# mohakbhardwaj/mjmpc

Hardware: AMD Instinct MI355X
Metric: particle-steps/sec (reacher_7dof-v0 MPPI 4096p x H32 per GPU, control loop incl. noise, rollout, update, shift) (higher is better)
Workload: dtype f64

## Files before the change

include/mjmpc_amd.h:

```cpp
#ifndef MJMPC_AMD_H
#define MJMPC_AMD_H

#include <stdint.h>

#ifdef __cplusplus
extern "C" {
#endif

#define MJMPC_ABI_VERSION 4

#define MJMPC_F32 0
#define MJMPC_F64 1

#define MJMPC_E_BADARG (-1)
#define MJMPC_E_BADMODEL (-2)
#define MJMPC_E_NOGPU (-3)

#define MJMPC_ARM_BLOB_LEN 255
#define MJMPC_ARM_STATE_LEN 19

typedef struct mjmpc_arm_s* mjmpc_arm_t;

int mjmpc_abi_version(void);
const char* mjmpc_last_error(void);
int mjmpc_device_count(void);
int mjmpc_graph_kernel_nodes(void* hip_graph, int64_t* n_out);
int mjmpc_graph_signature(void* hip_graph, uint64_t* n_out);

int mjmpc_arm_create(const double* model_blob, int n_blob, int device, mjmpc_arm_t* out);
int mjmpc_arm_destroy(mjmpc_arm_t h);
int mjmpc_arm_dims(mjmpc_arm_t h, int* nv, int* nu, int* d_obs);

int mjmpc_arm_set_shard_models(mjmpc_arm_t h, const double* model_blobs, int n_shards);

int mjmpc_arm_set_state(mjmpc_arm_t h, const double* qpos, const double* qvel, const double* target_pos,
                        void* stream);
int mjmpc_arm_set_shard_states(mjmpc_arm_t h, const double* states, int n_shards, void* stream);
double* mjmpc_arm_state_ptr(mjmpc_arm_t h);

int mjmpc_arm_rollout(mjmpc_arm_t h, int dtype, int64_t P, int H, const double* d_mean, const void* d_noise,
                      void* d_costs, void* d_actions, void* d_obs, void* d_next_obs, void* stream);

int mjmpc_arm_rollout_cl(mjmpc_arm_t h, int dtype, int64_t P, int H, const double* d_weights, const void* d_noise,
                         void* d_costs, void* d_actions, void* d_obs, void* d_next_obs, void* stream);

int mjmpc_arm_rollout_fused(mjmpc_arm_t h, int dtype, int64_t P, int H, const double* d_mean, const void* d_noise,
                            const double* d_filter_coeffs, const double* d_gseq, void* d_costs, void* d_actions,
                            double* d_q0, void* stream);

int mjmpc_arm_mppi_step(mjmpc_arm_t h, int dtype, int64_t P, int H, const double* d_mean, double* d_mean_out,
                        const double* d_gseq, const double* d_filter_coeffs, const double* d_chol, uint64_t seed,
                        uint64_t offset, int64_t particle_offset, int64_t* d_step_counter, double lam, double step_size,
                        int shift_mode, double* d_action_out, double* h_action_slots, double* d_record, int env_step,
                        void* d_step_cost, void* d_step_next_obs, void* d_costs, void* d_actions, double* d_q0, void* stream);

int mjmpc_arm_rollout_sampled(mjmpc_arm_t h, int dtype, int64_t P, int H, const double* d_mean, const double* d_gseq,
                              const double* d_filter_coeffs, const double* d_chol, int chol_full, uint64_t seed, uint64_t offset,
                              int64_t particle_offset, const int64_t* d_step_counter, void* d_costs, void* d_actions,
                              double* d_q0, void* stream);

int mjmpc_arm_mppi_combine(mjmpc_arm_t h, int dtype, const double* d_records, int n_records, int H, const double* d_mean,
                           double* d_mean_out, int64_t* d_step_counter, double step_size, int shift_mode,
                           double* d_action_out, double* h_action_slots, int env_step, void* d_step_cost,
                           void* d_step_next_obs, void* stream);

int mjmpc_arm_step_state(mjmpc_arm_t h, int dtype, const double* d_action, void* d_cost, void* d_next_obs,
                         void* stream);
int mjmpc_arm_get_state(mjmpc_arm_t h, double* qpos, double* qvel, void* stream);
int mjmpc_arm_rollout_fused_batch(mjmpc_arm_t h, int dtype, int64_t P_total, int H, const double* d_means, const void* d_noise,
                                  const double* d_filter_coeffs, const double* d_gseq, void* d_costs, void* d_actions,
                                  double* d_q0, void* stream);
int mjmpc_arm_rollout_fused_batch_obs(mjmpc_arm_t h, int dtype, int64_t P_total, int H, const double* d_means,
                                      const void* d_noise, const double* d_filter_coeffs, const double* d_gseq, void* d_costs,
                                      void* d_actions, double* d_q0, void* d_next_obs, void* stream);
int mjmpc_arm_step_shard_states(mjmpc_arm_t h, int dtype, const double* d_actions, void* d_costs, void* d_next_obs, void* stream);
int mjmpc_arm_get_shard_states(mjmpc_arm_t h, double* qpos, double* qvel, void* stream);

// ... 266 lines not shown
```

mjmpc_amd/_lib.py:

```python
import ctypes
import os
import threading

_HERE = os.path.dirname(os.path.abspath(__file__))
LIB_PATH = os.environ.get("MJMPC_AMD_LIB", os.path.join(_HERE, "libmjmpc_amd.so"))

F32, F64 = 0, 1
ABI_VERSION = 4

_vp = ctypes.c_void_p
_i64 = ctypes.c_int64
_int = ctypes.c_int
_dbl = ctypes.c_double
_dp = ctypes.POINTER(ctypes.c_double)

SIGNATURES = {
    "mjmpc_abi_version": (_int, []),
    "mjmpc_last_error": (ctypes.c_char_p, []),
    "mjmpc_device_count": (_int, []),
    "mjmpc_arm_create": (_int, [_dp, _int, _int, ctypes.POINTER(_vp)]),
    "mjmpc_arm_set_shard_models": (_int, [_vp, _dp, _int]),
    "mjmpc_arm_set_shard_states": (_int, [_vp, _dp, _int, _vp]),
    "mjmpc_arm_destroy": (_int, [_vp]),
    "mjmpc_arm_dims": (_int, [_vp, ctypes.POINTER(_int), ctypes.POINTER(_int), ctypes.POINTER(_int)]),
    "mjmpc_arm_set_state": (_int, [_vp, _dp, _dp, _dp, _vp]),
    "mjmpc_arm_state_ptr": (_vp, [_vp]),
    "mjmpc_arm_rollout": (_int, [_vp, _int, _i64, _int, _vp, _vp, _vp, _vp, _vp, _vp, _vp]),
    "mjmpc_arm_rollout_cl": (_int, [_vp, _int, _i64, _int, _vp, _vp, _vp, _vp, _vp, _vp, _vp]),
    "mjmpc_arm_rollout_fused": (_int, [_vp, _int, _i64, _int, _vp, _vp, _vp, _vp, _vp, _vp, _vp, _vp]),
    "mjmpc_tree_rollout_fused": (_int, [_vp, _int, _i64, _int, _vp, _vp, _vp, _vp, _vp, _vp, _vp, _vp]),
    "mjmpc_arm_step_state": (_int, [_vp, _int, _vp, _vp, _vp, _vp]),
    "mjmpc_arm_get_state": (_int, [_vp, _dp, _dp, _vp]),
    "mjmpc_arm_rollout_fused_batch": (_int, [_vp, _int, _i64, _int, _vp, _vp, _vp, _vp, _vp, _vp, _vp, _vp]),
    "mjmpc_arm_rollout_fused_batch_obs": (_int, [_vp, _int, _i64, _int, _vp, _vp, _vp, _vp, _vp, _vp, _vp, _vp, _vp]),
    "mjmpc_arm_step_shard_states": (_int, [_vp, _int, _vp, _vp, _vp, _vp]),
    "mjmpc_arm_get_shard_states": (_int, [_vp, _dp, _dp, _vp]),
    "mjmpc_arm_mppi_combine": (_int, [_vp, _int, _vp, _int, _int, _vp, _vp, _vp, ctypes.c_double, _int, _vp, _vp, _int, _vp, _vp, _vp]),
    "mjmpc_arm_rollout_sampled": (_int, [_vp, _int, _i64, _int, _vp, _vp, _vp, _vp, _int, ctypes.c_uint64, ctypes.c_uint64, _i64, _vp,
                                         _vp, _vp, _vp, _vp]),
    "mjmpc_arm_mppi_step": (_int, [_vp, _int, _i64, _int, _vp, _vp, _vp, _vp, _vp, ctypes.c_uint64, ctypes.c_uint64, _i64, _vp,
                                   _dbl, _dbl, _int, _vp, _vp, _vp, _int, _vp, _vp, _vp, _vp, _vp, _vp]),
    "mjmpc_tree_create": (_int, [_dp, _int, _int, ctypes.POINTER(_vp)]),
    "mjmpc_tree_create_ex": (_int, [_dp, _int, _int, _int, ctypes.POINTER(_vp)]),
    "mjmpc_tree_destroy": (_int, [_vp]),
    "mjmpc_tree_dims": (_int, [_vp, ctypes.POINTER(_int), ctypes.POINTER(_int), ctypes.POINTER(_int)]),
    "mjmpc_tree_nq": (_int, [_vp]),
    "mjmpc_tree_set_shard_models": (_int, [_vp, _dp, _int]),
    "mjmpc_tree_set_state": (_int, [_vp, _dp, _dp, _dp, _vp]),
    "mjmpc_tree_set_shard_states": (_int, [_vp, _dp, _int, _vp]),
    "mjmpc_tree_rollout": (_int, [_vp, _int, _i64, _int, _vp, _vp, _vp, _vp, _vp, _vp, _vp]),
    "mjmpc_tree_rollout_cl": (_int, [_vp, _int, _i64, _int, _vp, _vp, _vp, _vp, _vp, _vp, _vp]),
    "mjmpc_tree_step_state": (_int, [_vp, _int, _vp, _vp, _vp, _vp]),
    "mjmpc_tree_get_state": (_int, [_vp, _dp, _dp, _vp]),
    "mjmpc_tree_rollout_fused_batch": (_int, [_vp, _int, _i64, _int, _vp, _vp, _vp, _vp, _vp, _vp, _vp, _vp]),
    "mjmpc_tree_rollout_fused_batch_obs": (_int, [_vp, _int, _i64, _int, _vp, _vp, _vp, _vp, _vp, _vp, _vp, _vp, _vp]),
    "mjmpc_tree_step_shard_states": (_int, [_vp, _int, _vp, _vp, _vp, _vp]),
    "mjmpc_tree_get_shard_states": (_int, [_vp, _dp, _dp, _vp]),
    "mjmpc_tree_set_batch_models": (_int, [_vp, _dp, _int, _int]),
    "mjmpc_tree_set_env_model": (_int, [_vp, _dp]),
    "mjmpc_tree_solver_failures": (_int, [_vp, ctypes.POINTER(ctypes.c_uint32)]),
    "mjmpc_tree_diverged": (_int, [_vp, ctypes.POINTER(ctypes.c_uint32)]),
    "mjmpc_analytic_rollout": (_int, [_int, _vp, _int, _int, _vp, _int, _i64, _int, _vp, _vp, _vp, _vp, _vp, _vp, _int,
                                      _vp]),
    "mjmpc_arm_solver_failures": (_int, [_vp, ctypes.POINTER(ctypes.c_uint32)]),
# ... 181 lines not shown
```

mjmpc_amd/control/controller.py:

```python
import copy
import ctypes
import gc
import inspect
from abc import ABC, abstractmethod

import numpy as np

from .. import _lib
from ._device import DeviceUpdater
from .sharding import local_block
from .control_utils import generate_noise


def _seed_value(seed):
    if seed is None:
        seed = int(np.random.SeedSequence().generate_state(1)[0])
    if not isinstance(seed, (int, np.integer)) or seed < 0:
        raise ValueError("Seed must be a non-negative integer or omitted, not {}".format(seed))
    return int(seed)


class Controller(ABC):
    def __init__(self, d_state, d_obs, d_action, action_lows, action_highs, horizon, gamma, n_iters,
                 set_sim_state_fn=None, rollout_fn=None, sample_mode='mean', batch_size=1, seed=0,
# ... 314 lines not shown
        if self.noise_mode == 'device_mt19937':
            return self.dev.sample_noise_mt19937(n_loc, self._cov_host, self.filter_coeffs, self.seed_val, steps_ahead,
                                                 dtype=self.noise_dtype, d_step=self._step_dev, filtered=False,
                                                 particle_offset=self.dev.comm.rank * n_loc)
        return self.dev.sample_noise(n_loc, self._noise_cov(), self.filter_coeffs, self.seed_val, steps_ahead,
                                     dtype=self.noise_dtype, d_step=self._step_dev, filtered=False,
                                     particle_offset=self.dev.comm.rank * n_loc,
                                     device_cov_diagonal=self.cov_type == 'diagonal')

    def _noise_cov(self):
        return self._cov_host if self._static_cov() else None

    def _bind_mono(self, env_step, direct=False):
        n_loc = self.local_particles
        chol, coeffs, _ = self.dev.prepare_noise(self._cov_host, self.filter_coeffs)
        fc = np.asarray(self.filter_coeffs, np.float64)
        coeffs = None if (fc[0] == 1.0 and fc[1] == 0.0 and fc[2] == 0.0) else coeffs
        eng = getattr(self._rollout_fn, "engine", None)
        post = self._graph_post
        own_step = post is not None and getattr(post, "__self__", None) is eng and getattr(post, "__name__", "") == "step_state"
        sharded = self.dev.comm.world_size > 1
        self._mono_rec = self.dev.record("fused_rec", 2 + self.horizon * self.d_action) if sharded else None
        self._mono_steps_env = bool(env_step and own_step)
        self._mono_launch, self._mono_combine = {}, {}
        recs = self.dev.comm.all_gather(self._mono_rec) if sharded else None
        self._mono_gather = None
        if sharded:
            mk = getattr(self.dev.comm, "all_gather_launcher", None)
            self._mono_gather = mk(self._mono_rec) if (mk and direct) else (lambda: self.dev.comm.all_gather(self._mono_rec))
        for src, dst in ((self.dev.mean, self.dev.mean_alt), (self.dev.mean_alt, self.dev.mean)):
            self._mono_launch[id(src)], _ = self._rollout_fn.mono_launcher(
                n_loc, self.horizon, src, dst, self.dev.gseq, coeffs, chol, self.seed_val, 0, self.dev.comm.rank * n_loc,
                self._step_dev, self.lam, self.step_size, _SHIFT_MODES[self.base_action], action_out=self._action_dev,
                action_slots=None if sharded else self._action_pin, record=self._mono_rec,
                env_step=self._mono_steps_env and not sharded,
                bind_stream=direct or not sharded)
            if sharded:
                self._mono_combine[id(src)] = self._rollout_fn.combine_launcher(
                    recs, recs.shape[0], self.horizon, src, dst, self._step_dev, self.step_size,
                    _SHIFT_MODES[self.base_action], self._action_dev, self._action_pin, self._mono_steps_env)

    def _noise_ahead(self):
        return ((not self._mono) and self._graph_on and self.noise_mode == 'device'
                and (self._fused_capable() or (self._cem_fused() and not self._cem_in_kernel())))

    def _cem_in_kernel(self):
        eng = getattr(self._rollout_fn, "engine", None)
        return (self._cem_fused() and getattr(self, "_want_cem_in_kernel", True) and hasattr(self._rollout_fn, "sampled")
                and hasattr(eng, "mppi_step_supported") and eng.mppi_step_supported(self.local_particles, self.horizon)
                and getattr(eng, "num_shards", 1) == 1 and not getattr(eng, "_per_shard_states", False)
                and not hasattr(eng, "shard_blobs") and getattr(eng, "dtype", self.noise_dtype) == self.noise_dtype)

    def _cem_fused(self):
        return False

    def _mono_capable(self):
        if not (getattr(self, "_want_mono", True) and self._graph_on and self.noise_mode == 'device' and self.n_iters == 1
                and self._fused_capable() and self._static_cov() and hasattr(self._rollout_fn, "mono")):
            return False
# ... 107 lines not shown
            self._step_host = self.num_steps
            self._action_dev = torch.zeros(self.d_action, dtype=torch.float64, device=self.dev.device)
            self._action_pin = torch.zeros(2 * (self.d_action + 1), dtype=torch.float64).pin_memory()
            self._action_np = self._action_pin.numpy()
            if self._mono and (self.dev.comm.world_size == 1 or getattr(self.dev.comm, "lib_collectives", False)):
                self._bind_mono(env_step=True, direct=True)
                self._graph = "direct"
                self.launch_mode = "launched directly"
            else:
                self._capture_iteration()
        if self._graph is None:
            return self._optimize_eager_after_fallback(state)
        if self._step_host != self.num_steps:
            if self._ahead:
                raise RuntimeError("num_steps was changed while an iteration enqueued ahead was in flight")
            self._step_dev.fill_(self.num_steps)
            self._noise_valid = False
        if not self._noise_valid:
            if self._noise_ahead():
                self._draw_raw(self.local_particles, 0)
            elif self._cem_in_kernel():
                self.dev.factor_cov(self.filter_coeffs)
            self._noise_valid = True
        replay = self._device_iteration if self._graph == "direct" else self._graph.replay
        if self._ahead == 0:
            self._action_np[self._slot(self.num_steps) + self.d_action] = -1.0
            replay()
            self._ahead = 1
        if self._lookahead and self._mono and self.dev.comm.world_size == 1:
            self._action_np[self._slot(self.num_steps + 1) + self.d_action] = -1.0
            replay()
            self._ahead += 1
        action = self._wait_action()
        self._ahead -= 1
        self.num_steps += 1
        self._step_host = self.num_steps
        self._mean_stale = True
        if not self._static_cov():
            self._cov_stale = True
        return action, 0.0

    def _capture_iteration(self):
        torch = self.dev.torch
        sharded_mono = self._mono and self.dev.comm.world_size > 1
        if self._mono:
            self._bind_mono(env_step=False)
# ... 39 lines not shown
                    self._device_iteration()
                self._graph = self._tape_or_graph(g, tape, cap_stream)
            else:
                g = torch.cuda.CUDAGraph()
                with torch.cuda.graph(g):
                    self._device_iteration()
                self._graph = g
        except Exception as e:
            err = e
        finally:
            if gc_was_on:
                gc.enable()
        if not self.dev.comm.all_agree(err is None, self.dev.device):
            import warnings
            warnings.warn("hipGraph capture of the control iteration failed (%s); running eagerly"
                          % (err if err is not None else "on another rank",))
            torch.cuda.synchronize(self.dev.device)
            self.dev.mean.copy_(keep[0])
            self.dev.cov.copy_(keep[2])
            self._graph_on = False
            self._graph = None
            self.graph_fallback = True
            self._mono = False
            self._mono_launch, self._mono_combine = {}, {}

    def _tape_or_graph(self, g, tape, cap_stream):
        torch = self.dev.torch
        self.launch_mode = "hipGraph replay"
        try:
            t = _LaunchTape(tape, cap_stream, self.dev)
            g2 = torch.cuda.CUDAGraph(keep_graph=True)
            with torch.cuda.graph(g2):
                t.replay()
            n1, n2 = (ctypes.c_int64 * 2)(), (ctypes.c_int64 * 2)()
            _lib.check(self.dev.lib.mjmpc_graph_kernel_nodes(ctypes.c_void_p(int(g.raw_cuda_graph())), n1))
            _lib.check(self.dev.lib.mjmpc_graph_kernel_nodes(ctypes.c_void_p(int(g2.raw_cuda_graph())), n2))
            s1, s2 = (ctypes.c_uint64 * 2)(), (ctypes.c_uint64 * 2)()
            _lib.check(self.dev.lib.mjmpc_graph_signature(ctypes.c_void_p(int(g.raw_cuda_graph())), s1))
            _lib.check(self.dev.lib.mjmpc_graph_signature(ctypes.c_void_p(int(g2.raw_cuda_graph())), s2))
            del g2
            if n1[0] > 0 and n1[0] == n2[0] and n1[1] == n2[1] and s1[0] == s2[0] and s1[1] == s2[1]:
                self.launch_mode = "launch tape (%d calls, %d kernels)" % (len(t.calls), n1[0])
                return t
        except Exception as e:
            import warnings
            warnings.warn("launch tape not available (%s); replaying the hipGraph" % (e,))
        g.instantiate()
# ... 57 lines not shown
```

mjmpc_amd/csrc/arm_rollout.hip:

```cpp
#include <hip/hip_runtime.h>

#include <cstdlib>
#include <type_traits>

#include "arm_model.h"
#include "arm_rollout.h"
#include "lanegroup.h"
#include "noise_device.h"

namespace mjmpc {
namespace {

template <typename T>
constexpr int newton_maxit() { return sizeof(T) == 4 ? 32 : 12; }

#define PHASE() asm volatile("" ::: "memory")
#define LDS_WAVE_SYNC()                                        \
    do {                                                       \
        __builtin_amdgcn_fence(__ATOMIC_ACQ_REL, "wavefront"); \
        asm volatile("" ::: "memory");                         \
        __builtin_amdgcn_sched_barrier(0);                     \
    } while (0)

constexpr int N_LINK_FIELDS = O_NV / LANES;
// ... 1331 lines not shown
            const unsigned long long mine = particle_lanes(lane);
            const double* rst = record();
            if (rst == nullptr) {
            } else if (__ballot(mj_is_bad(x)) & mine) {
                q = (T)rst[l8];
                v = (T)rst[LANES + l8];
                sq = (T)rst[2 * LANES + 3 + l8];
                cq = (T)rst[3 * LANES + 3 + l8];
                aw = T(0);
                const int f0 = rflags<ROLE>(ldsM);
                rflags_set<ROLE>(ldsM, f0 | 1 | 4 | RST_EVER);
                if (role_counts<ROLE>() && diag && l8 == 0 && rc->count) { atomicAdd(diag + 1, 1u); if (f0 & RST_REAL) atomicAdd(diag + 2, 1u); }
            } else if (bal & mine) {
                rflags_set<ROLE>(ldsM, rflags<ROLE>(ldsM) | 2);
            }
        }
    }
    LDS_WAVE_SYNC();
    ST.mark(13);
}

constexpr int MONO_RED = 32;

template <typename T, bool DUO, typename MT>
__device__ __forceinline__ void real_env_step(const MT& M, const ArmInts& I, const MonoStep& mo, double* st, T q, T v,
                                              const T* tgt, const double* action, int A, T* lds, int lane, int wave, int l8,
                                              int g, unsigned* diag) {
    const int nv = I.nv;
    T* ldsM = lds + g * PSTRIDE;
    T aw = T(0);
    if (l8 >= nv) { q = T(0); v = T(0); }
    T sinq, cosq;
    sincos_(q, sinq, cosq);
    if constexpr (XJ) { if (M.xj_slide()) { sinq = T(0); cosq = T(1); } }
    int rows = 0;
    Stamps ST;
    ST.begin();
    bool fs = false;
    ResetCtl rc;
    rc.count = g == 0;
    if (DUO && wave == 1) rflags_set<SOLVE>(ldsM, RST_REAL);
    else rflags_set<SOLO>(ldsM, RST_REAL);
    auto record = [&mo]() -> const double* { return mo.reset_rec; };
    if (mo.reset_rec) {
        if (DUO && wave == 1) reset_check_start<SOLVE>(rc, q, v, lane, ldsM);
        else reset_check_start<SOLO>(rc, q, v, lane, ldsM);
    }
    if (DUO && wave == 1) {
        if constexpr (DUO) {
            T nosite[3];
            for (int sub = 0; sub < I.frame_skip; ++sub) {
                arm_front<SOLVE>(M, I, q, v, aw, sinq, cosq, rows, T(0), ldsM, lane, l8, nosite, diag, fs, ST, &rc);
                arm_back<SOLVE>(M, q, v, aw, sinq, cosq, ldsM, l8, fs, ST, lane, &rc, nullptr, record);
            }
        }
        return;
    }
    constexpr int R = DUO ? DYN : SOLO;
    const T u = l8 < A ? (T)action[l8] : T(0);
    const T tau_act = M.link(O_GEAR) * fmin(fmax(u, M.link(O_CTRL_LO)), M.link(O_CTRL_HI));
    T site[3];
    unsigned* dcount = diag;
    for (int sub = 0; sub < I.frame_skip; ++sub) {
        if (R == DYN && sub > 0) arm_back<R>(M, q, v, aw, sinq, cosq, ldsM, l8, fs, ST, lane, &rc, dcount, record);
        arm_front<R>(M, I, q, v, aw, sinq, cosq, rows, tau_act, ldsM, lane, l8, site, dcount, fs, ST, &rc);
        if constexpr (R == SOLO) arm_back<R>(M, q, v, aw, sinq, cosq, ldsM, l8, fs, ST, lane, &rc, dcount, record);
    }
    const int site_lane = lane_of_link(lane, I.site_link);
    for (int k = 0; k < 3; ++k) site[k] = __shfl(site[k], site_lane);
    if constexpr (R == DYN) arm_back<R>(M, q, v, aw, sinq, cosq, ldsM, l8, fs, ST, lane, &rc, dcount, record);
    if (rc.any && (rflags<R>(ldsM) & 4))
        for (int k = 0; k < 3; ++k) site[k] = (T)mo.reset_rec[2 * LANES + k];
    if (g == 0) {
        const T dx = site[0] - tgt[0], dy = site[1] - tgt[1], dz = site[2] - tgt[2];
        if (mo.step_cost && l8 == 0)
            ((T*)mo.step_cost)[0] = fabs(dx) + fabs(dy) + fabs(dz) + T(5) * sqrt_(dx * dx + dy * dy + dz * dz);
        if (mo.step_nobs) {
            T* o = (T*)mo.step_nobs;
            if (l8 < nv) { o[l8] = q; o[nv + l8] = v; }
            if (l8 < 3) {
                const T hh = l8 == 0 ? site[0] : (l8 == 1 ? site[1] : site[2]);
                const T gg = l8 == 0 ? tgt[0] : (l8 == 1 ? tgt[1] : tgt[2]);
// ... 16 lines not shown
        const double q = red[tid], x = q == INFINITY ? -INFINITY : (-1.0 / lam) * q;
        double m = x;
        for (int o = 1; o < LANES; o <<= 1) m = fmax(m, __shfl_xor(m, o));
        const double e = x == -INFINITY ? 0.0 : exp(x - m);
        double S = e;
        for (int o = 1; o < LANES; o <<= 1) S += __shfl_xor(S, o);
        red[LANES + tid] = e;
        if (tid == 0) { rec_out[0] = m; rec_out[1] = S; }
    }
    __syncthreads();
    double e[LANES];
#pragma unroll
    for (int k = 0; k < LANES; ++k) e[k] = red[LANES + k];
    for (int j = tid; j < HA; j += NT) {
        double acc = 0.0;
#pragma unroll
        for (int k = 0; k < LANES; ++k) acc += e[k] * (double)actT[k * HA + j];
        rec_out[2 + j] = acc;
    }
}

constexpr int MAX_A = 8;
constexpr int FIN_CHUNK = 4;
#ifdef MJMPC_ARM_XJ
#define MJMPC_FINISH_WAVES __attribute__((amdgpu_waves_per_eu(1, 1)))
#else
#define MJMPC_FINISH_WAVES
#endif
template <typename T>
__global__ __launch_bounds__(128) MJMPC_FINISH_WAVES void arm_mppi_finish_kernel(const T* __restrict__ model, const double* __restrict__ recs, long n_rec,
                                                              int H, int A, const double* __restrict__ mean_in,
                                                              double* __restrict__ mean_out, const MonoStep mo,
                                                              int env_step, unsigned* diag) {
    __shared__ __attribute__((aligned(16))) T lds[LANES * PSTRIDE + ARM_BLOB_LEN + 3];
    __shared__ double sh[2 * (2 + MAX_A)];
    const int tid = threadIdx.x, t = blockIdx.x, HA = H * A, rec = 2 + HA;
    const int lane = tid & 63, wave = __builtin_amdgcn_readfirstlane(tid >> 6);
    const bool stepper = t == 0 && env_step && mo.state_io && !mo.record;
    double rm[FIN_CHUNK], rs[FIN_CHUNK], rw[FIN_CHUNK][MAX_A];
    auto fetch = [&](long base) {
#pragma unroll
        for (int k = 0; k < FIN_CHUNK; ++k) {
            const long b = base + tid + 128L * k;
            const double* r = recs + (b < n_rec ? b : 0) * rec;
            rm[k] = b < n_rec ? r[0] : -INFINITY;
            rs[k] = r[1];
#pragma unroll
            for (int a = 0; a < MAX_A; ++a) rw[k][a] = a < A ? r[2 + t * A + a] : 0.0;
        }
    };
    fetch(0);
    const double mean_old = (tid < A && !mo.record) ? mean_in[t * A + tid] : 0.0;
    const long long count = (t == 0 && mo.step_counter) ? *mo.step_counter : 0;
    const int l8 = lane_link(lane), g = lane_slot(lane);
    T q0 = T(0), v0 = T(0), tgt[3] = {T(0), T(0), T(0)};
    if (stepper) {
        for (int k = tid; k < ARM_BLOB_LEN; k += 128) lds[LANES * PSTRIDE + k] = model[k];
        for (int k = tid; k < LANES * PSTRIDE; k += 128) lds[k] = T(0);
        q0 = (T)mo.state_io[l8];
        v0 = (T)mo.state_io[LANES + l8];
        for (int k = 0; k < 3; ++k) tgt[k] = (T)mo.state_io[2 * LANES + k];
    }
    double m = -INFINITY, S = 0.0, W[MAX_A];
#pragma unroll
    for (int a = 0; a < MAX_A; ++a) W[a] = 0.0;
    for (long base = 0; base < n_rec; base += 128L * FIN_CHUNK) {
        if (base > 0) fetch(base);
        double mn = m;
#pragma unroll
        for (int k = 0; k < FIN_CHUNK; ++k) mn = fmax(mn, rm[k]);
        const double sc = m == -INFINITY ? 0.0 : exp(m - mn);
        S *= sc;
#pragma unroll
        for (int a = 0; a < MAX_A; ++a) W[a] *= sc;
#pragma unroll
        for (int k = 0; k < FIN_CHUNK; ++k) {
            const double c = rm[k] == -INFINITY ? 0.0 : exp(rm[k] - mn);
            S += c * rs[k];
#pragma unroll
            for (int a = 0; a < MAX_A; ++a) W[a] += c * rw[k][a];
        }
        m = mn;
    }
    double M = m;
    for (int o = 32; o > 0; o >>= 1) M = fmax(M, __shfl_xor(M, o));
    if (lane == 0) sh[wave] = M;
    __syncthreads();
    M = fmax(sh[0], sh[1]);
    const double f = m == -INFINITY ? 0.0 : exp(m - M);
    S *= f;
    for (int o = 32; o > 0; o >>= 1) S += __shfl_xor(S, o);
#pragma unroll
    for (int a = 0; a < MAX_A; ++a) {
        W[a] *= f;
        for (int o = 32; o > 0; o >>= 1) W[a] += __shfl_xor(W[a], o);
    }
    __syncthreads();
    if (lane == 0) {
        sh[wave * (2 + MAX_A) + 1] = S;
#pragma unroll
        for (int a = 0; a < MAX_A; ++a) sh[wave * (2 + MAX_A) + 2 + a] = W[a];
    }
    __syncthreads();
    S = sh[1] + sh[(2 + MAX_A) + 1];
    const double wsum = tid < A ? sh[2 + tid] + sh[(2 + MAX_A) + 2 + tid] : 0.0;
    if (mo.record) {
        if (tid < A) mo.record[2 + t * A + tid] = wsum;
        if (t == 0 && tid == 0) { mo.record[0] = M; mo.record[1] = S; }
        return;
    }
    double nm = 0.0;
    if (tid < A) {
        nm = (1.0 - mo.step_size) * mean_old + mo.step_size * (wsum / S);
        if (mo.shift_mode < 0) {
            mean_out[t * A + tid] = nm;
        } else {
            if (t > 0) mean_out[(t - 1) * A + tid] = nm;
            if (t == H - 1) mean_out[t * A + tid] = mo.shift_mode == 0 ? 0.0 : nm;
        }
    }
    if (t != 0) return;
    __syncthreads();
    if (tid < A) sh[tid] = nm;
    double* slot = mo.action_host ? mo.action_host + (count & 1) * (A + 1) : nullptr;
    if (tid < A) {
        if (mo.action_out) mo.action_out[tid] = nm;
        if (slot) __hip_atomic_store(slot + tid, nm, __ATOMIC_RELAXED, __HIP_MEMORY_SCOPE_SYSTEM);
    }
    if (wave == 0) {
        asm volatile("s_waitcnt vmcnt(0)" ::: "memory");
        if (tid == 0) {
            if (mo.step_counter) *mo.step_counter = count + 1;
            if (slot) __hip_atomic_store(slot + A, (double)(count + 1), __ATOMIC_RELAXED, __HIP_MEMORY_SCOPE_SYSTEM);
        }
    }
    if (!stepper) return;
    __syncthreads();
    Model<T, true> Mv{lds + LANES * PSTRIDE, l8};
    Mv.cache();
    ArmInts I;
    I.site_link = (int)lds[LANES * PSTRIDE + O_SITE_LINK];
    I.n_sphere = (int)lds[LANES * PSTRIDE + O_N_SPHERE];
    I.sph_link = (int)lds[LANES * PSTRIDE + O_SPH_LINK];
    I.frame_skip = (int)lds[LANES * PSTRIDE + O_FRAME_SKIP];
    I.nv = (int)lds[LANES * PSTRIDE + O_NV];
    I.site_link = __builtin_amdgcn_readfirstlane(I.site_link);
    I.n_sphere = __builtin_amdgcn_readfirstlane(I.n_sphere);
    I.sph_link = __builtin_amdgcn_readfirstlane(I.sph_link);
    I.frame_skip = __builtin_amdgcn_readfirstlane(I.frame_skip);
    I.nv = __builtin_amdgcn_readfirstlane(I.nv);
    real_env_step<T, true>(Mv, I, mo, mo.state_io, q0, v0, tgt, sh, A, lds, lane, wave, l8, g, diag);
}


template <typename T, bool STEP, bool CL, int WAVES, bool DUO, bool MONO, bool EB = false>
__global__ __launch_bounds__(DUO ? 128 : 64) __attribute__((amdgpu_waves_per_eu(WAVES, WAVES))) void arm_rollout_kernel(const T* __restrict__ model, const double* state,
                                                         long P, int H, int A, const double* mean,
                                                         const T* __restrict__ noise, T* __restrict__ cost,
                                                         T* __restrict__ act, T* __restrict__ obs,
                                                         T* __restrict__ nobs, double* state_out, unsigned* diag,
                                                         RolloutFusion fuse, const MonoStep mono_arg) {
    const MonoStep* mop = &mono_arg;
    constexpr int SHAPE = DUO ? 2 : 1, NW = SHAPE;
    constexpr bool QUAD = false;
    const qflag_ptr qf = nullptr;
    int seq = 0;
#include "arm_rollout_body.inc"
}
template <typename T, int NW, bool MONO, bool EB = false>
__global__ __launch_bounds__(64 * NW) __attribute__((amdgpu_waves_per_eu(1, 1))) void arm_rollout_flags_kernel(const T* __restrict__ model, const double* state,
                                                         long P, int H, int A, const double* mean,
                                                         const T* __restrict__ noise, T* __restrict__ cost,
                                                         T* __restrict__ act, T* __restrict__ obs,
                                                         T* __restrict__ nobs, unsigned* diag,
// ... 1 lines not shown
    const MonoStep* mop = &mono_arg;
    constexpr int SHAPE = 10 + NW;
    constexpr bool STEP = false, CL = false, DUO = false, QUAD = true;
    double* const state_out = nullptr;
    __shared__ int qflags[QF_COUNT];
    qflag_ptr qf = (qflag_ptr)qflags;
    int seq = 0;
#include "arm_rollout_body.inc"
}
}

#ifdef MJMPC_ARM_XJ
#define launch_arm_mppi_finish launch_arm_mppi_finish_xj
#define launch_arm_rollout launch_arm_rollout_xj
#else
long arm_rollout_groups(long P) { return (P + LANES - 1) / LANES; }
long mono_record_doubles(long groups, int H, int A) { return groups * (2 + (long)H * A); }
#endif

template <typename T>
hipError_t launch_arm_mppi_finish(const T* model, const double* records, long n_rec, int H, int A, const double* mean_in,
                                  double* mean_out, const MonoStep& mono, int env_step, unsigned* diag, hipStream_t stream) {
    if (A > MAX_A || H < 1 || n_rec < 1) return hipErrorInvalidValue;
    hipLaunchKernelGGL(arm_mppi_finish_kernel<T>, dim3((unsigned)H), dim3(128), 0, stream, model, records, n_rec, H, A, mean_in,
                       mean_out, mono, env_step, diag);
    return hipGetLastError();
}
template hipError_t launch_arm_mppi_finish<float>(const float*, const double*, long, int, int, const double*, double*,
                                                  const MonoStep&, int, unsigned*, hipStream_t);
template hipError_t launch_arm_mppi_finish<double>(const double*, const double*, long, int, int, const double*, double*,
                                                   const MonoStep&, int, unsigned*, hipStream_t);

template <typename T>
hipError_t launch_arm_rollout(const T* model, const double* state, long P, int H, int A, const double* mean,
                              const T* noise, T* cost, T* act, T* obs, T* nobs, double* state_out,
                              unsigned* diag, hipStream_t stream, RolloutFusion fuse,
                              const MonoStep* mono, int eb) {
    if (P <= 0 || H <= 0) return hipSuccess;
    if (eb && (XJ || mono || fuse.clw || obs || fuse.state_shard_size <= 0 || fuse.shard_size > 0)) return hipErrorInvalidValue;
    if (eb == 1 && (state_out || fuse.state_shard_size % LANES != 0 || P % fuse.state_shard_size != 0)) return hipErrorInvalidValue;
    if (eb == 2 && (!state_out || H != 1 || noise || act || fuse.state_shard_size != LANES)) return hipErrorInvalidValue;
    const unsigned grid = eb == 2 ? (unsigned)P : (unsigned)((P + LANES - 1) / LANES);
    int dev = 0, cus = 256;
    if (hipGetDevice(&dev) == hipSuccess) hipDeviceGetAttribute(&cus, hipDeviceAttributeMultiprocessorCount, dev);
    const long simds = 4L * cus;
    const int cap = ((long)grid <= 2 * simds || sizeof(T) == 8) ? 2 : 3;
    static const int duo_env = [] { const char* e = getenv("MJMPC_ARM_DUO"); return e ? atoi(e) : -1; }();
// ... 74 lines not shown
```

mjmpc_amd/csrc/capi.hip:

```cpp
#include <hip/hip_runtime.h>

#include <algorithm>
#include <climits>
#include <cmath>
#include <cstdarg>
#include <cstdio>
#include <cstring>
#include <type_traits>
#include <vector>

#include "../../include/mjmpc_amd.h"
#include "arm_model.h"
#include "analytic_rollout.h"
#include "arm_rollout.h"
#include "noise_mt.h"
#include "tree_model.h"
#include "tree_rollout.h"
#include "update.h"

constexpr size_t MJMPC_DIAG_BYTES = 8 * (2 + 64);

namespace {

thread_local char g_err[512] = "";

// ... 712 lines not shown
    mo.action_out = d_action_out;
    mo.action_host = h_action_slots;
    mo.step_counter = (long long*)d_step_counter;
    mo.record = d_record;
    mo.state_io = h->state;
    mo.step_cost = d_step_cost;
    mo.step_nobs = d_step_next_obs;
    mo.reset_rec = h->reset_rec;
    const int do_env = (env_step && !d_record) ? 1 : 0;
    mjmpc::RolloutFusion fuse = arm_fuse(h);
    fuse.filt = d_filter_coeffs;
    fuse.gseq = d_gseq;
    fuse.q0_out = d_q0;
    return with_dtype(dtype, "arm_mppi_step launch", [&](auto tag) {
        using T = decltype(tag);
        hipError_t e = arm_rollout_launch<T>(h, model<T>(h), h->state, (long)P, H, h->nu, d_mean, nullptr, (T*)d_costs,
                                             (T*)d_actions, nullptr, nullptr, nullptr, h->diag, s, fuse, &mo);
        if (e == hipSuccess && !rollout_only)
            e = arm_finish_launch<T>(h, model<T>(h), h->mono_tree, groups, H, h->nu, d_mean, d_mean_out, mo, do_env, h->diag, s);
        return e;
    });
}

int mjmpc_arm_rollout_sampled(mjmpc_arm_t h, int dtype, int64_t P, int H, const double* d_mean, const double* d_gseq,
                              const double* d_filter_coeffs, const double* d_chol, int chol_full, uint64_t seed, uint64_t offset,
                              int64_t particle_offset, const int64_t* d_step_counter, void* d_costs, void* d_actions,
                              double* d_q0, void* stream) {
    if (!h || !d_mean || !d_gseq || !d_chol) return fail(MJMPC_E_BADARG, "null argument");
    if (P < 1 || H < 1) return fail(MJMPC_E_BADARG, "P and H must be positive");
    if (h->n_shards > 1 || h->n_state_shards > 1)
        return fail(MJMPC_E_BADARG, "sampled rollouts run one model and one start state (no per-shard blocks)");
    HIP_TRY(hipSetDevice(h->device));
    hipStream_t s = (hipStream_t)stream;
    const long groups = mjmpc::arm_rollout_groups((long)P);
    if (int rc = arm_grow_mono(h, (size_t)mjmpc::mono_record_doubles(groups, H, h->nu), s)) return rc;
    mjmpc::MonoStep mo;
    mo.chol = d_chol;
    mo.chol_full = chol_full ? 1 : 0;
    mo.seed = seed;
    mo.offset = offset;
    mo.particle_offset = (long)particle_offset;
    mo.d_step = (const long long*)d_step_counter;
    mo.lam = 1.0;
    mo.shift_mode = -2;
    mo.tree = h->mono_tree;
    mjmpc::RolloutFusion fuse = arm_fuse(h);
// ... 996 lines not shown
```

mjmpc_amd/envs/arm_engine.py:

```python
import numpy as np

from .. import _lib
from ..models.compile import ArmModel, compile_arm
from ._engine import (RolloutEngine, SimulationUnstableError, _ptr, _torch,
                      make_device_rollout_fn, make_rollout_fn)


class ArmRolloutEngine(RolloutEngine):
    _abi = "arm"
    _model_type, _compile = ArmModel, staticmethod(compile_arm)
    _layout = (19, 8, 16)

    def _create(self, blob, n_blob, device, h_out):
        return self._lib.mjmpc_arm_create(blob, n_blob, device, h_out)

    def _unpack(self, state):
        return self._checked_state(state["qp"], state["qv"], state["target_pos"])

    def _start_qpos(self):
        return np.zeros(self.model.nv)

    def _overrides(self, rand):
        if any(np.any(np.asarray(v) != 0) for v in rand.get("dof_frictionloss", {}).values()):
            raise NotImplementedError("a non-zero dof_frictionloss adds friction-loss constraint rows, which the "
# ... 17 lines not shown
                        particle_offset, step_counter, q0_out=None):
        self._refuse_with_terms("rollout_sampled")
        P, H, A = int(num_particles), int(horizon), self.d_action
        costs, act = self._buffer("costs", (P, H)), self._buffer("act", (P, H, A))
        q0 = self._q0_buffer(P, q0_out)
        _lib.check(self._lib.mjmpc_arm_rollout_sampled(self._h, self._code, P, H, _ptr(mean), _ptr(gamma_seq), _ptr(filter_coeffs),
                                                       _ptr(chol), int(bool(chol_full)), int(seed) & (2 ** 64 - 1), int(offset),
                                                       int(particle_offset), _ptr(step_counter), _ptr(costs), _ptr(act), _ptr(q0),
                                                       self._stream()))
        return costs, act, q0

    def mppi_step(self, num_particles, horizon, mean, mean_out, gamma_seq, filter_coeffs, chol, seed, offset,
                  particle_offset, step_counter, lam, step_size, shift_mode, action_out=None, action_slots=None, record=None,
                  env_step=False, want_trajectories=False):
        self._refuse_with_terms("mppi_step")
        launch, out = self.mppi_step_launcher(num_particles, horizon, mean, mean_out, gamma_seq, filter_coeffs, chol, seed,
                                              offset, particle_offset, step_counter, lam, step_size, shift_mode, action_out,
                                              action_slots, record, env_step, want_trajectories)
        launch()
        return out

    def mppi_step_launcher(self, num_particles, horizon, mean, mean_out, gamma_seq, filter_coeffs, chol, seed, offset,
                           particle_offset, step_counter, lam, step_size, shift_mode, action_out=None, action_slots=None,
                           record=None, env_step=False, want_trajectories=False, bind_stream=True):
        self._refuse_with_terms("mppi_step_launcher")
        P, H, A = int(num_particles), int(horizon), self.d_action
        costs = act = q0 = None
        if want_trajectories:
            costs, act, q0 = self._buffer("costs", (P, H)), self._buffer("act", (P, H, A)), self._q0_buffer(P)
        scost = self._buffer("step_cost", (1,)) if env_step else None
        snobs = self._buffer("step_obs", (self.d_obs,)) if env_step else None
        keep = (mean, mean_out, gamma_seq, filter_coeffs, chol, step_counter, action_out, action_slots, record, scost, snobs,
                costs, act, q0)
        args = (self._h, self._code, P, H, _ptr(mean), _ptr(mean_out), _ptr(gamma_seq), _ptr(filter_coeffs), _ptr(chol),
                int(seed) & (2 ** 64 - 1), int(offset), int(particle_offset), _ptr(step_counter), float(lam), float(step_size),
                int(shift_mode), _ptr(action_out), _ptr(action_slots), _ptr(record), int(bool(env_step)), _ptr(scost),
                _ptr(snobs), _ptr(costs), _ptr(act), _ptr(q0))
        fn, check, stream = self._lib.mjmpc_arm_mppi_step, _lib.check, self._stream
        if bind_stream:
            args = args + (stream(),)

            def launch(_keep=keep):
                check(fn(*args))
        else:
            def launch(_keep=keep):
                check(fn(*args, stream()))

        return launch, ((costs, act, q0) if want_trajectories else None)

    def mppi_combine_launcher(self, records, n_records, horizon, mean, mean_out, step_counter, step_size, shift_mode,
                              action_out, action_slots, env_step):
        self._refuse_with_terms("mppi_combine_launcher")
        scost = self._buffer("step_cost", (1,))
        snobs = self._buffer("step_obs", (self.d_obs,))
        keep = (records, mean, mean_out, step_counter, action_out, action_slots, scost, snobs)
        args = (self._h, self._code, _ptr(records), int(n_records), int(horizon), _ptr(mean), _ptr(mean_out),
                _ptr(step_counter), float(step_size), int(shift_mode), _ptr(action_out), _ptr(action_slots),
                int(bool(env_step)), _ptr(scost), _ptr(snobs))
        fn, check, stream = self._lib.mjmpc_arm_mppi_combine, _lib.check, self._stream

        def launch(_keep=keep):
# ... 4 lines not shown
```

Measured before the change: 684.4 million.

## Split MPPI finish into publisher and stepper blocks, add host spin-wait step path

The finish kernel gains an extra block that publishes the action to pinned host slots while block 0 runs the real environment step concurrently, with model and state loads hoisted before the reductions. The reductions now use DPP row operations across eight rows instead of wave shuffles with several __syncthreads. A new C API entry launches the step and spin-waits on the pinned host flag, so the controller can return the action without a full stream sync. This adds host CPU spinning and more complex kernel control flow.

```diff
diff --git a/include/mjmpc_amd.h b/include/mjmpc_amd.h
--- a/include/mjmpc_amd.h
+++ b/include/mjmpc_amd.h
@@ -15,6 +15,7 @@
 #define MJMPC_E_BADARG (-1)
 #define MJMPC_E_BADMODEL (-2)
 #define MJMPC_E_NOGPU (-3)
+#define MJMPC_E_TIMEOUT (-4)
 
 #define MJMPC_ARM_BLOB_LEN 255
 #define MJMPC_ARM_STATE_LEN 19
@@ -53,6 +54,13 @@
                         uint64_t offset, int64_t particle_offset, int64_t* d_step_counter, double lam, double step_size,
                         int shift_mode, double* d_action_out, double* h_action_slots, double* d_record, int env_step,
                         void* d_step_cost, void* d_step_next_obs, void* d_costs, void* d_actions, double* d_q0, void* stream);
+
+int mjmpc_arm_mppi_step_wait(mjmpc_arm_t h, int dtype, int64_t P, int H, const double* d_mean, double* d_mean_out,
+                             const double* d_gseq, const double* d_filter_coeffs, const double* d_chol, uint64_t seed,
+                             uint64_t offset, int64_t particle_offset, int64_t* d_step_counter, double lam, double step_size,
+                             int shift_mode, double* d_action_out, double* h_action_slots, double* d_record, int env_step,
+                             void* d_step_cost, void* d_step_next_obs, void* d_costs, void* d_actions, double* d_q0, void* stream,
+                             int64_t step, double* h_action);
 
 int mjmpc_arm_rollout_sampled(mjmpc_arm_t h, int dtype, int64_t P, int H, const double* d_mean, const double* d_gseq,
                               const double* d_filter_coeffs, const double* d_chol, int chol_full, uint64_t seed, uint64_t offset,
diff --git a/mjmpc_amd/_lib.py b/mjmpc_amd/_lib.py
--- a/mjmpc_amd/_lib.py
+++ b/mjmpc_amd/_lib.py
@@ -40,6 +40,8 @@
                                          _vp, _vp, _vp, _vp]),
     "mjmpc_arm_mppi_step": (_int, [_vp, _int, _i64, _int, _vp, _vp, _vp, _vp, _vp, ctypes.c_uint64, ctypes.c_uint64, _i64, _vp,
                                    _dbl, _dbl, _int, _vp, _vp, _vp, _int, _vp, _vp, _vp, _vp, _vp, _vp]),
+    "mjmpc_arm_mppi_step_wait": (_int, [_vp, _int, _i64, _int, _vp, _vp, _vp, _vp, _vp, ctypes.c_uint64, ctypes.c_uint64, _i64, _vp,
+                                        _dbl, _dbl, _int, _vp, _vp, _vp, _int, _vp, _vp, _vp, _vp, _vp, _vp, _i64, _vp]),
     "mjmpc_tree_create": (_int, [_dp, _int, _int, ctypes.POINTER(_vp)]),
     "mjmpc_tree_create_ex": (_int, [_dp, _int, _int, _int, ctypes.POINTER(_vp)]),
     "mjmpc_tree_destroy": (_int, [_vp]),
diff --git a/mjmpc_amd/control/controller.py b/mjmpc_amd/control/controller.py
--- a/mjmpc_amd/control/controller.py
+++ b/mjmpc_amd/control/controller.py
@@ -360,7 +360,7 @@
         sharded = self.dev.comm.world_size > 1
         self._mono_rec = self.dev.record("fused_rec", 2 + self.horizon * self.d_action) if sharded else None
         self._mono_steps_env = bool(env_step and own_step)
-        self._mono_launch, self._mono_combine = {}, {}
+        self._mono_launch, self._mono_combine, self._mono_wait = {}, {}, {}
         recs = self.dev.comm.all_gather(self._mono_rec) if sharded else None
         self._mono_gather = None
         if sharded:
@@ -373,6 +373,11 @@
                 action_slots=None if sharded else self._action_pin, record=self._mono_rec,
                 env_step=self._mono_steps_env and not sharded,
                 bind_stream=direct or not sharded)
+            if direct and not sharded:
+                self._mono_wait[id(src)], _ = self._rollout_fn.mono_launcher(
+                    n_loc, self.horizon, src, dst, self.dev.gseq, coeffs, chol, self.seed_val, 0, self.dev.comm.rank * n_loc,
+                    self._step_dev, self.lam, self.step_size, _SHIFT_MODES[self.base_action], action_out=self._action_dev,
+                    action_slots=self._action_pin, env_step=self._mono_steps_env, wait=True)
             if sharded:
                 self._mono_combine[id(src)] = self._rollout_fn.combine_launcher(
                     recs, recs.shape[0], self.horizon, src, dst, self._step_dev, self.step_size,
@@ -526,6 +531,16 @@
             elif self._cem_in_kernel():
                 self.dev.factor_cov(self.filter_coeffs)
             self._noise_valid = True
+        if (self._graph == "direct" and self._ahead == 0 and not self._lookahead
+                and (self._graph_post is None or self._mono_steps_env)):
+            step_and_wait = self._mono_wait.get(id(self.dev.mean))
+            if step_and_wait is not None:
+                action = step_and_wait(self.num_steps)
+                self.dev.mean, self.dev.mean_alt = self.dev.mean_alt, self.dev.mean
+                self.num_steps += 1
+                self._step_host = self.num_steps
+                self._mean_stale = True
+                return action, 0.0
         replay = self._device_iteration if self._graph == "direct" else self._graph.replay
         if self._ahead == 0:
             self._action_np[self._slot(self.num_steps) + self.d_action] = -1.0
@@ -611,7 +626,7 @@
             self._graph = None
             self.graph_fallback = True
             self._mono = False
-            self._mono_launch, self._mono_combine = {}, {}
+            self._mono_launch, self._mono_combine, self._mono_wait = {}, {}, {}
 
     def _tape_or_graph(self, g, tape, cap_stream):
         torch = self.dev.torch
diff --git a/mjmpc_amd/csrc/arm_rollout.hip b/mjmpc_amd/csrc/arm_rollout.hip
--- a/mjmpc_amd/csrc/arm_rollout.hip
+++ b/mjmpc_amd/csrc/arm_rollout.hip
@@ -1377,30 +1377,40 @@
 
 constexpr int MONO_RED = 32;
 
+
+template <typename T, typename MT>
+__device__ __forceinline__ void real_env_state(const MT& M, int nv, int l8, T& q, T& v, T& sinq, T& cosq) {
+    if (l8 >= nv) { q = T(0); v = T(0); }
+    sincos_(q, sinq, cosq);
+    if constexpr (XJ) { if (M.xj_slide()) { sinq = T(0); cosq = T(1); } }
+}
+
+template <typename T, bool DUO>
+__device__ __forceinline__ ResetCtl real_env_flags(const MonoStep& mo, T q, T v, T* lds, int lane, int wave, int g) {
+    T* ldsM = lds + g * PSTRIDE;
+    ResetCtl rc;
+    rc.count = g == 0;
+    if (DUO && wave == 1) rflags_set<SOLVE>(ldsM, RST_REAL);
+    else rflags_set<SOLO>(ldsM, RST_REAL);
+    if (mo.reset_rec) {
+        if (DUO && wave == 1) reset_check_start<SOLVE>(rc, q, v, lane, ldsM);
+        else reset_check_start<SOLO>(rc, q, v, lane, ldsM);
+    }
+    return rc;
+}
+
 template <typename T, bool DUO, typename MT>
-__device__ __forceinline__ void real_env_step(const MT& M, const ArmInts& I, const MonoStep& mo, double* st, T q, T v,
-                                              const T* tgt, const double* action, int A, T* lds, int lane, int wave, int l8,
+__device__ __forceinline__ void real_env_step(const MT& M, const ArmInts& I, const MonoStep& mo, double* st, T q, T v, T sinq,
+                                              T cosq, const T* tgt, T u, ResetCtl rc, T* lds, int lane, int wave, int l8,
                                               int g, unsigned* diag) {
     const int nv = I.nv;
     T* ldsM = lds + g * PSTRIDE;
     T aw = T(0);
-    if (l8 >= nv) { q = T(0); v = T(0); }
-    T sinq, cosq;
-    sincos_(q, sinq, cosq);
-    if constexpr (XJ) { if (M.xj_slide()) { sinq = T(0); cosq = T(1); } }
     int rows = 0;
     Stamps ST;
     ST.begin();
     bool fs = false;
-    ResetCtl rc;
-    rc.count = g == 0;
-    if (DUO && wave == 1) rflags_set<SOLVE>(ldsM, RST_REAL);
-    else rflags_set<SOLO>(ldsM, RST_REAL);
     auto record = [&mo]() -> const double* { return mo.reset_rec; };
-    if (mo.reset_rec) {
-        if (DUO && wave == 1) reset_check_start<SOLVE>(rc, q, v, lane, ldsM);
-        else reset_check_start<SOLO>(rc, q, v, lane, ldsM);
-    }
     if (DUO && wave == 1) {
         if constexpr (DUO) {
             T nosite[3];
@@ -1412,7 +1422,6 @@
         return;
     }
     constexpr int R = DUO ? DYN : SOLO;
-    const T u = l8 < A ? (T)action[l8] : T(0);
     const T tau_act = M.link(O_GEAR) * fmin(fmax(u, M.link(O_CTRL_LO)), M.link(O_CTRL_HI));
     T site[3];
     unsigned* dcount = diag;
@@ -1475,6 +1484,27 @@
 
 constexpr int MAX_A = 8;
 constexpr int FIN_CHUNK = 4;
+constexpr int FIN_ROWS = 8;
+__device__ __forceinline__ double row_max16(double x) {
+    x = fmax(x, dpp_all<0xB1>(x));
+    x = fmax(x, dpp_all<0x4E>(x));
+    x = fmax(x, dpp_all<0x124>(x));
+    return fmax(x, dpp_all<0x128>(x));
+}
+__device__ __forceinline__ double row_sum16(double x) {
+    x += dpp_all<0xB1>(x);
+    x += dpp_all<0x4E>(x);
+    x += dpp_all<0x124>(x);
+    return x + dpp_all<0x128>(x);
+}
+#ifdef MJMPC_STAMPS
+#define FIN_MARK(k) do { if (diag && tid == 0 && (blockIdx.x == 0 || publisher)) \
+        ((unsigned long long*)diag)[2 + 48 + (blockIdx.x == 0 ? 0 : 8) + (k)] = wall_clock64(); } while (0)
+#define FIN_DRAIN() asm volatile("s_waitcnt vmcnt(0)" ::: "memory")
+#else
+#define FIN_MARK(k) do { } while (0)
+#define FIN_DRAIN() do { } while (0)
+#endif
 #ifdef MJMPC_ARM_XJ
 #define MJMPC_FINISH_WAVES __attribute__((amdgpu_waves_per_eu(1, 1)))
 #else
@@ -1486,10 +1516,32 @@
                                                               double* __restrict__ mean_out, const MonoStep mo,
                                                               int env_step, unsigned* diag) {
     __shared__ __attribute__((aligned(16))) T lds[LANES * PSTRIDE + ARM_BLOB_LEN + 3];
-    __shared__ double sh[2 * (2 + MAX_A)];
-    const int tid = threadIdx.x, t = blockIdx.x, HA = H * A, rec = 2 + HA;
+    __shared__ double sh_m[FIN_ROWS], sh_p[FIN_ROWS][1 + MAX_A];
+    const bool split = env_step && mo.state_io && !mo.record;
+    const bool publisher = split && (int)blockIdx.x == H, stepper = split && blockIdx.x == 0;
+    const int tid = threadIdx.x, t = publisher ? 0 : blockIdx.x, HA = H * A, rec = 2 + HA;
     const int lane = tid & 63, wave = __builtin_amdgcn_readfirstlane(tid >> 6);
-    const bool stepper = t == 0 && env_step && mo.state_io && !mo.record;
+    if ((int)blockIdx.x >= H && !publisher) return;
+    FIN_MARK(0);
+    const int l8 = lane_link(lane), g = lane_slot(lane);
+    T q0 = T(0), v0 = T(0), sq0 = T(0), cq0 = T(1), tgt[3] = {T(0), T(0), T(0)};
+    Model<T, true> Mg{model, l8};
+    ArmInts I = {0, 0, 0, 0, 0};
+    static_assert(ARM_BLOB_LEN <= 256, "two scalars of the model block per thread");
+    T blob0 = T(0), blob1 = T(0);
+    if (stepper) {
+        blob0 = model[tid];
+        if (tid + 128 < ARM_BLOB_LEN) blob1 = model[tid + 128];
+        Mg.cache();
+        I.site_link = __builtin_amdgcn_readfirstlane((int)model[O_SITE_LINK]);
+        I.n_sphere = __builtin_amdgcn_readfirstlane((int)model[O_N_SPHERE]);
+        I.sph_link = __builtin_amdgcn_readfirstlane((int)model[O_SPH_LINK]);
+        I.frame_skip = __builtin_amdgcn_readfirstlane((int)model[O_FRAME_SKIP]);
+        I.nv = __builtin_amdgcn_readfirstlane((int)model[O_NV]);
+        q0 = (T)mo.state_io[l8];
+        v0 = (T)mo.state_io[LANES + l8];
+        for (int k = 0; k < 3; ++k) tgt[k] = (T)mo.state_io[2 * LANES + k];
+    }
     double rm[FIN_CHUNK], rs[FIN_CHUNK], rw[FIN_CHUNK][MAX_A];
     auto fetch = [&](long base) {
 #pragma unroll
@@ -1504,15 +1556,13 @@
     };
     fetch(0);
     const double mean_old = (tid < A && !mo.record) ? mean_in[t * A + tid] : 0.0;
-    const long long count = (t == 0 && mo.step_counter) ? *mo.step_counter : 0;
-    const int l8 = lane_link(lane), g = lane_slot(lane);
-    T q0 = T(0), v0 = T(0), tgt[3] = {T(0), T(0), T(0)};
+    const bool publishes = t == 0 && !stepper;
+    const long long count = (publishes && mo.step_counter) ? *mo.step_counter : 0;
     if (stepper) {
-        for (int k = tid; k < ARM_BLOB_LEN; k += 128) lds[LANES * PSTRIDE + k] = model[k];
+        lds[LANES * PSTRIDE + tid] = blob0;
+        if (tid + 128 < ARM_BLOB_LEN) lds[LANES * PSTRIDE + tid + 128] = blob1;
         for (int k = tid; k < LANES * PSTRIDE; k += 128) lds[k] = T(0);
-        q0 = (T)mo.state_io[l8];
-        v0 = (T)mo.state_io[LANES + l8];
-        for (int k = 0; k < 3; ++k) tgt[k] = (T)mo.state_io[2 * LANES + k];
+        real_env_state(Mg, I.nv, l8, q0, v0, sq0, cq0);
     }
     double m = -INFINITY, S = 0.0, W[MAX_A];
 #pragma unroll
@@ -1535,28 +1585,36 @@
         }
         m = mn;
     }
-    double M = m;
-    for (int o = 32; o > 0; o >>= 1) M = fmax(M, __shfl_xor(M, o));
-    if (lane == 0) sh[wave] = M;
-    __syncthreads();
-    M = fmax(sh[0], sh[1]);
+    FIN_DRAIN();
+    FIN_MARK(1);
+    const int row = wave * 4 + (lane >> 4);
+    const bool row_head = (lane & 15) == 0;
+    double M = row_max16(m);
+    if (row_head) sh_m[row] = M;
+    duo_barrier();
+    M = sh_m[0];
+#pragma unroll
+    for (int r = 1; r < FIN_ROWS; ++r) M = fmax(M, sh_m[r]);
     const double f = m == -INFINITY ? 0.0 : exp(m - M);
-    S *= f;
-    for (int o = 32; o > 0; o >>= 1) S += __shfl_xor(S, o);
+    S = row_sum16(S * f);
+    if (row_head) sh_p[row][0] = S;
 #pragma unroll
     for (int a = 0; a < MAX_A; ++a) {
-        W[a] *= f;
-        for (int o = 32; o > 0; o >>= 1) W[a] += __shfl_xor(W[a], o);
-    }
-    __syncthreads();
-    if (lane == 0) {
-        sh[wave * (2 + MAX_A) + 1] = S;
-#pragma unroll
-        for (int a = 0; a < MAX_A; ++a) sh[wave * (2 + MAX_A) + 2 + a] = W[a];
-    }
-    __syncthreads();
-    S = sh[1] + sh[(2 + MAX_A) + 1];
-    const double wsum = tid < A ? sh[2 + tid] + sh[(2 + MAX_A) + 2 + tid] : 0.0;
+        if (a < A) {
+            W[a] = row_sum16(W[a] * f);
+            if (row_head) sh_p[row][1 + a] = W[a];
+        }
+    }
+    ResetCtl rc;
+    if (stepper) rc = real_env_flags<T, true>(mo, q0, v0, lds, lane, wave, g);
+    duo_barrier();
+    S = sh_p[0][0];
+    double wsum = tid < A ? sh_p[0][1 + tid] : 0.0;
+#pragma unroll
+    for (int r = 1; r < FIN_ROWS; ++r) {
+        S += sh_p[r][0];
+        if (tid < A) wsum += sh_p[r][1 + tid];
+    }
     if (mo.record) {
         if (tid < A) mo.record[2 + t * A + tid] = wsum;
         if (t == 0 && tid == 0) { mo.record[0] = M; mo.record[1] = S; }
@@ -1565,44 +1623,39 @@
     double nm = 0.0;
     if (tid < A) {
         nm = (1.0 - mo.step_size) * mean_old + mo.step_size * (wsum / S);
-        if (mo.shift_mode < 0) {
+        if (publisher) {
+        } else if (mo.shift_mode < 0) {
             mean_out[t * A + tid] = nm;
         } else {
             if (t > 0) mean_out[(t - 1) * A + tid] = nm;
             if (t == H - 1) mean_out[t * A + tid] = mo.shift_mode == 0 ? 0.0 : nm;
         }
     }
+    FIN_MARK(2);
     if (t != 0) return;
-    __syncthreads();
-    if (tid < A) sh[tid] = nm;
-    double* slot = mo.action_host ? mo.action_host + (count & 1) * (A + 1) : nullptr;
-    if (tid < A) {
-        if (mo.action_out) mo.action_out[tid] = nm;
-        if (slot) __hip_atomic_store(slot + tid, nm, __ATOMIC_RELAXED, __HIP_MEMORY_SCOPE_SYSTEM);
-    }
-    if (wave == 0) {
+    if (publishes) {
+        if (wave != 0) return;
+        double* slot = mo.action_host ? mo.action_host + (count & 1) * (A + 1) : nullptr;
+        if (tid < A) {
+            if (mo.action_out) mo.action_out[tid] = nm;
+            if (slot) __hip_atomic_store(slot + tid, nm, __ATOMIC_RELAXED, __HIP_MEMORY_SCOPE_SYSTEM);
+        }
+        FIN_MARK(3);
         asm volatile("s_waitcnt vmcnt(0)" ::: "memory");
+        FIN_MARK(4);
         if (tid == 0) {
             if (mo.step_counter) *mo.step_counter = count + 1;
             if (slot) __hip_atomic_store(slot + A, (double)(count + 1), __ATOMIC_RELAXED, __HIP_MEMORY_SCOPE_SYSTEM);
         }
-    }
-    if (!stepper) return;
-    __syncthreads();
-    Model<T, true> Mv{lds + LANES * PSTRIDE, l8};
-    Mv.cache();
-    ArmInts I;
-    I.site_link = (int)lds[LANES * PSTRIDE + O_SITE_LINK];
-    I.n_sphere = (int)lds[LANES * PSTRIDE + O_N_SPHERE];
-    I.sph_link = (int)lds[LANES * PSTRIDE + O_SPH_LINK];
-    I.frame_skip = (int)lds[LANES * PSTRIDE + O_FRAME_SKIP];
-    I.nv = (int)lds[LANES * PSTRIDE + O_NV];
-    I.site_link = __builtin_amdgcn_readfirstlane(I.site_link);
-    I.n_sphere = __builtin_amdgcn_readfirstlane(I.n_sphere);
-    I.sph_link = __builtin_amdgcn_readfirstlane(I.sph_link);
-    I.frame_skip = __builtin_amdgcn_readfirstlane(I.frame_skip);
-    I.nv = __builtin_amdgcn_readfirstlane(I.nv);
-    real_env_step<T, true>(Mv, I, mo, mo.state_io, q0, v0, tgt, sh, A, lds, lane, wave, l8, g, diag);
+        return;
+    }
+    const double ua = __shfl(nm, l8);
+    const T u = l8 < A ? (T)ua : T(0);
+    Model<T, true> Mv = Mg;
+    Mv.m = lds + LANES * PSTRIDE;
+    FIN_MARK(5);
+    real_env_step<T, true>(Mv, I, mo, mo.state_io, q0, v0, sq0, cq0, tgt, u, rc, lds, lane, wave, l8, g, diag);
+    FIN_MARK(6);
 }
 
 
@@ -1650,7 +1703,8 @@
 hipError_t launch_arm_mppi_finish(const T* model, const double* records, long n_rec, int H, int A, const double* mean_in,
                                   double* mean_out, const MonoStep& mono, int env_step, unsigned* diag, hipStream_t stream) {
     if (A > MAX_A || H < 1 || n_rec < 1) return hipErrorInvalidValue;
-    hipLaunchKernelGGL(arm_mppi_finish_kernel<T>, dim3((unsigned)H), dim3(128), 0, stream, model, records, n_rec, H, A, mean_in,
+    const unsigned grid = (unsigned)H + ((env_step && mono.state_io && !mono.record) ? 1u : 0u);
+    hipLaunchKernelGGL(arm_mppi_finish_kernel<T>, dim3(grid), dim3(128), 0, stream, model, records, n_rec, H, A, mean_in,
                        mean_out, mono, env_step, diag);
     return hipGetLastError();
 }
diff --git a/mjmpc_amd/csrc/capi.hip b/mjmpc_amd/csrc/capi.hip
--- a/mjmpc_amd/csrc/capi.hip
+++ b/mjmpc_amd/csrc/capi.hip
@@ -1,6 +1,7 @@
 #include <hip/hip_runtime.h>
 
 #include <algorithm>
+#include <chrono>
 #include <climits>
 #include <cmath>
 #include <cstdarg>
@@ -759,6 +760,53 @@
     });
 }
 
+static inline double slot_flag_load(const double* p) {
+    uint64_t b = __atomic_load_n((const uint64_t*)p, __ATOMIC_ACQUIRE);
+    double v;
+    std::memcpy(&v, &b, sizeof(v));
+    return v;
+}
+static inline void slot_flag_store(double* p, double v) {
+    uint64_t b;
+    std::memcpy(&b, &v, sizeof(b));
+    __atomic_store_n((uint64_t*)p, b, __ATOMIC_RELEASE);
+}
+static inline void spin_pause() { __builtin_ia32_pause(); }
+
+int mjmpc_arm_mppi_step_wait(mjmpc_arm_t h, int dtype, int64_t P, int H, const double* d_mean, double* d_mean_out,
+                             const double* d_gseq, const double* d_filter_coeffs, const double* d_chol, uint64_t seed,
+                             uint64_t offset, int64_t particle_offset, int64_t* d_step_counter, double lam, double step_size,
+                             int shift_mode, double* d_action_out, double* h_action_slots, double* d_record, int env_step,
+                             void* d_step_cost, void* d_step_next_obs, void* d_costs, void* d_actions, double* d_q0, void* stream,
+                             int64_t step, double* h_action) {
+    if (!h || !h_action_slots || !h_action || !d_step_counter)
+        return fail(MJMPC_E_BADARG, "null argument (the pinned action slots, the caller's action buffer and the step counter are required)");
+    if (d_record || shift_mode == -2) return fail(MJMPC_E_BADARG, "an iteration that publishes no action (d_record / shift_mode -2) cannot be waited for");
+    if (step < 0) return fail(MJMPC_E_BADARG, "step %lld", (long long)step);
+    const int A = h->nu;
+    double* slot = h_action_slots + (step & 1) * (A + 1);
+    const double want = (double)(step + 1);
+    slot_flag_store(slot + A, -1.0);
+    if (int rc = mjmpc_arm_mppi_step(h, dtype, P, H, d_mean, d_mean_out, d_gseq, d_filter_coeffs, d_chol, seed, offset,
+                                     particle_offset, d_step_counter, lam, step_size, shift_mode, d_action_out, h_action_slots,
+                                     d_record, env_step, d_step_cost, d_step_next_obs, d_costs, d_actions, d_q0, stream))
+        return rc;
+    bool seen = false;
+    const auto t0 = std::chrono::steady_clock::now();
+    for (long spins = 1;; ++spins) {
+        if (slot_flag_load(slot + A) == want) { seen = true; break; }
+        spin_pause();
+        if ((spins & 0xFFF) == 0 && std::chrono::steady_clock::now() - t0 > std::chrono::seconds(1)) break;
+    }
+    if (!seen) {
+        HIP_TRY(hipStreamSynchronize((hipStream_t)stream));
+        if (slot_flag_load(slot + A) != want)
+            return fail(MJMPC_E_TIMEOUT, "the control iteration of step %lld finished without publishing its action", (long long)step);
+    }
+    std::memcpy(h_action, slot, sizeof(double) * A);
+    return 0;
+}
+
 int mjmpc_arm_rollout_sampled(mjmpc_arm_t h, int dtype, int64_t P, int H, const double* d_mean, const double* d_gseq,
                               const double* d_filter_coeffs, const double* d_chol, int chol_full, uint64_t seed, uint64_t offset,
                               int64_t particle_offset, const int64_t* d_step_counter, void* d_costs, void* d_actions,
diff --git a/mjmpc_amd/envs/arm_engine.py b/mjmpc_amd/envs/arm_engine.py
--- a/mjmpc_amd/envs/arm_engine.py
+++ b/mjmpc_amd/envs/arm_engine.py
@@ -63,7 +63,7 @@
 
     def mppi_step_launcher(self, num_particles, horizon, mean, mean_out, gamma_seq, filter_coeffs, chol, seed, offset,
                            particle_offset, step_counter, lam, step_size, shift_mode, action_out=None, action_slots=None,
-                           record=None, env_step=False, want_trajectories=False, bind_stream=True):
+                           record=None, env_step=False, want_trajectories=False, bind_stream=True, wait=False):
         self._refuse_with_terms("mppi_step_launcher")
         P, H, A = int(num_particles), int(horizon), self.d_action
         costs = act = q0 = None
@@ -78,6 +78,17 @@
                 int(shift_mode), _ptr(action_out), _ptr(action_slots), _ptr(record), int(bool(env_step)), _ptr(scost),
                 _ptr(snobs), _ptr(costs), _ptr(act), _ptr(q0))
         fn, check, stream = self._lib.mjmpc_arm_mppi_step, _lib.check, self._stream
+        if wait:
+            if action_slots is None or record is not None or not bind_stream:
+                raise ValueError("wait=True needs the pinned action slots and a bound stream, and publishes no record")
+            fnw, buf = self._lib.mjmpc_arm_mppi_step_wait, np.empty(A, np.float64)
+            args, out = args + (stream(),), buf.ctypes.data
+
+            def launch_wait(step, _keep=keep):
+                check(fnw(*args, step, out))
+                return buf.copy()
+
+            return launch_wait, ((costs, act, q0) if want_trajectories else None)
         if bind_stream:
             args = args + (stream(),)
 
```

After: 668.7 million. -2.3%, worse.
